# Fabstir/fabstir-vectordb

Measured on AMD Instinct MI355X. Metric: k-NN queries/sec at recall@10>=0.95, 1Mx384 f32, higher is better.
Workload: dtype f32

## Files before the change

### fabstir-vectordb_amd/csrc/fvdb_graph.cpp

```cpp
#include <algorithm>
#include <chrono>
#include <cstdio>
#include <cstdlib>
#include <cstring>
#include <map>
#include <new>
#include <string>
#include <vector>

#include "fvdb_internal.h"
#include "common.h"
#include "kernels_graph.h"
#include "kernels_graph_fast.h"
#include "kernels_graph_build.h"
#include "kernels_graph_maint.h"

using namespace fvdb;

struct fvdb_graph {
  fvdb_store* store = nullptr;
  uint32_t M = 0, M0 = 0;
  uint32_t stride0 = 0, strideU = 0;
  uint32_t n = 0, n_cap = 0;
  uint32_t u_rows = 0, u_cap = 0;
// ... 290 lines not shown
    g->tag += 1;
    hipLaunchKernelGGL(kernels.commit, dim3(1), dim3(kBuildThreads), lds, stream, v, first, n, grp.count, g->tag, 0u, nullptr, nullptr, nullptr, 1u);
    return;
  }
  for (uint32_t p = 0; p < grp.count; ++p) {
    g->tag += 1;
    hipLaunchKernelGGL(kernels.search, dim3(sched.K, kBuildLayers), dim3(kBuildThreads), lds, stream, v, first, n, sched.exact_positions,
                       g->tag, g->d_spec.as<uint32_t>(), g->d_elog.as<uint32_t>());
    hipLaunchKernelGGL(kernels.commit, dim3(1), dim3(kBuildThreads), lds, stream, v, first, n, sched.K, g->tag, sched.knobs.max_rerun,
                       g->d_spec.as<uint32_t>(), g->d_elog.as<uint32_t>(), g->d_chg.as<uint32_t>(), sched.knobs.strict);
  }
}

#ifdef FVDB_BUILD_STAMPS
void build_stamps_begin(fvdb_graph* g, BuildView* v) {
  (void)g->d_build_stamps.ensure(64 * 8);
  (void)hipMemset(g->d_build_stamps.p, 0, 64 * 8);
  v->dbg = g->d_build_stamps.as<unsigned long long>();
}
void build_stamps_print(fvdb_graph* g, const BuildState& st, uint32_t done) {
  unsigned long long h[16] = {};
  (void)hipMemcpy(h, g->d_build_stamps.p, sizeof(h), hipMemcpyDeviceToHost);
  fprintf(stderr, "[build stamps] of replay+select (us): replay %.1f  select %.1f  (table = the rest) | admissions %.1f\n", h[6] * 0.01 / std::max(1u, st.n_rerun),
          h[7] * 0.01 / std::max(1u, st.n_rerun), (double)h[8] / std::max(1u, st.n_rerun));
  const double us = 0.01, nn = std::max(1u, st.n_rerun);
  fprintf(stderr, "[build stamps] per searched insert (us): replay+select %.1f  fetch %.1f  score %.1f | greedy %.1f  all searches %.1f  links %.1f"
          " | rounds %.1f expanded %.1f scored %.0f\n", h[0] * us / nn, h[1] * us / nn, h[2] * us / nn, h[3] * us / nn, h[4] * us / nn,
          h[5] * us / std::max(1u, done), st.rounds / nn, st.consumed / nn, st.scored / nn);
}
#else
inline void build_stamps_begin(fvdb_graph*, BuildView*) {}
inline void build_stamps_print(fvdb_graph*, const BuildState&, uint32_t) {}
#endif

void report_insert(const InsertPlan& plan, const BuildState& st) {
  if (!getenv("FVDB_BUILD_DEBUG")) return;
  fprintf(stderr, "[device insert] %u linked, %u adopted, stops %u: entry %u, gave-up %u, order/strict %u, caps %u, added node nearer than a later pop %u, added node inside the final set %u, dropped node matters %u | "
          "checks %u, touched rows %u\n", st.cursor, st.n_valid, st.n_stopped, st.why[1], st.why[2], st.why[3], st.why[4], st.why[5], st.why[6],
          st.why[9], st.why[7], st.why[8]);
  fprintf(stderr, "[device insert] searches that left the register set: pops tied %u, evictions tied %u, result tied %u, heap overflow %u | speculations given up or restarted %u\n",
          st.why[11], st.why[12], st.why[13], st.why[14], st.spec_ties);
  fprintf(stderr, "[device insert] second looks: overlapping %u, nodes the popped newcomer would bring in %u, later pop is the maximum %u\n", st.why[15], st.why[16], st.why[17]);
  if (plan.repr == 2)
    fprintf(stderr, "[device insert] hashed visited set, %u slots: %u searches gave up on a full set (%u of them inserts handed to the host), "
            "entries after a search: largest %u, mean %.0f over %u searches\n", plan.slots, st.why[18], st.vis_host, st.vis_peak,
            (double)st.vis_sum / std::max(1u, st.vis_searches), st.vis_searches);
}

void fold_insert(fvdb_graph* g, const InsertPlan& plan, const BuildState& st, uint32_t launches, uint32_t* n_done,
                 fvdb_graph_insert_stats* stats) {
  if (plan.repr == 2) {
    g->ins_hashed += st.cursor;
    g->ins_vis_over += st.vis_host;
    g->ins_vis_searches += st.vis_searches;
    g->ins_vis_entries += st.vis_sum;
    g->ins_vis_peak = std::max(g->ins_vis_peak, st.vis_peak);
  }
  g->entry = st.entry;
  g->top_level = st.entry_level;
  g->has_entry = st.has_entry != 0;
  const fvdb_graph_insert_stats acc{st.cursor, st.status, st.n_valid, st.n_rerun, st.n_stopped, st.rounds, st.consumed, st.scored, st.ties, launches};
  g->last = acc;
  if (stats) *stats = acc;
  if (n_done) *n_done = st.cursor;
}

using FastKernel = decltype(&hnsw_search_fast_kernel<3, 16, true>);
template <int NB, int R>
FastKernel fast_kernel_of(bool bytemap) {
  return bytemap ? hnsw_search_fast_kernel<NB, R, true> : hnsw_search_fast_kernel<NB, R, false>;
}
FastKernel fast_kernel(uint32_t nb128, int R, bool bytemap) {
  switch (nb128) {
    case 1: return fast_kernel_of<1, 16>(bytemap);
    case 2: return fast_kernel_of<2, 16>(bytemap);
    case 3: return R == 8 ? fast_kernel_of<3, 8>(bytemap) : R == 12 ? fast_kernel_of<3, 12>(bytemap) : fast_kernel_of<3, 16>(bytemap);
    case 4: return fast_kernel_of<4, 12>(bytemap);
    case 5:
    case 6: return fast_kernel_of<6, 8>(bytemap);
    default: return fast_kernel_of<8, 6>(bytemap);
  }
}

struct SearchPlan {
  bool bytemap;
  uint32_t words, vstride, tcap, spill_cap, cand_cap;
  size_t lds;
  uint32_t wave_lds;
  FastKernel fast;
  decltype(&hnsw_search_kernel<true>) exact;
  bool rh;
};

int search_scratch(fvdb_graph* g, fvdb_ctx* ctx, uint32_t slot, uint32_t B, uint32_t ef, SearchPlan* sp) {
  sp->words = (g->n + 31) / 32;
  sp->tcap = getenv("FVDB_GRAPH_TCAP") ? std::max(1, atoi(getenv("FVDB_GRAPH_TCAP"))) : 8192;
  static const bool no_bytes = getenv("FVDB_GRAPH_BITMAP") != nullptr;
  const uint32_t vbytes = ((g->n + 63) / 64) * 64;
  sp->bytemap = !no_bytes && (uint64_t)vbytes * std::max<uint32_t>(B, 1024) <= (1ull << 30);
  sp->vstride = sp->bytemap ? vbytes : sp->words * 4;
  if (sp->words != g->vis_words || sp->tcap != g->vis_tcap || sp->vstride != g->vis_stride) {
    for (auto& v : g->vis_B) v = 0;
    g->vis_words = sp->words;
    g->vis_tcap = sp->tcap;
    g->vis_stride = sp->vstride;
  }
  if (B > g->vis_B[slot]) {
    HIPCHK(ctx, g->s_visited[slot].ensure((size_t)B * sp->vstride));
    HIPCHK(ctx, hipMemsetAsync(g->s_visited[slot].p, 0, g->s_visited[slot].cap, ctx->stream));
    HIPCHK(ctx, g->s_touched[slot].ensure((size_t)B * sp->tcap * 4));
    g->vis_B[slot] = B;
  }
  sp->spill_cap = std::min<uint32_t>(((g->n + 63) / 64) * 64, 8192);
  HIPCHK(ctx, g->s_spill[slot].ensure((size_t)B * sp->spill_cap * 8));
  const int cand_env = getenv("FVDB_GRAPH_CAND_CAP") ? atoi(getenv("FVDB_GRAPH_CAND_CAP")) : 0;
  sp->cand_cap = cand_env > 0 ? (uint32_t)cand_env : std::max<uint32_t>(1024, 8 * ef);
  sp->lds = graph_lds_bytes(g->store->dpad, ef, sp->cand_cap);
  if (sp->lds > 160 * 1024) FAIL(ctx, FVDB_E_UNSUPPORTED, "dimension / ef too large for the on-chip traversal state");
  return FVDB_OK;
}

int search_kernel(fvdb_graph* g, fvdb_ctx* ctx, uint32_t ef, SearchPlan* sp) {
  static const bool lds_heaps = getenv("FVDB_GRAPH_LDS_HEAPS") != nullptr;
  sp->rh = ef <= 63 && !lds_heaps;
  static const bool no_fast = getenv("FVDB_GRAPH_NO_FAST") != nullptr;
  static const int fast_r = getenv("FVDB_GRAPH_FAST_R") ? atoi(getenv("FVDB_GRAPH_FAST_R")) : 0;
  const uint32_t nb128 = (g->store->dpad + 127) / 128;
  if (no_fast || !sp->rh || nb128 > 8 || g->n >= 0x80000000u) {
    sp->exact = sp->rh ? hnsw_search_kernel<true> : hnsw_search_kernel<false>;
    return FVDB_OK;
  }
  int R = nb128 <= 3 ? 16 : (nb128 == 4 ? 12 : (nb128 <= 6 ? 8 : 6));
  if (nb128 == 3 && (fast_r == 8 || fast_r == 12)) R = fast_r;
  sp->wave_lds = (uint32_t)((std::max(graph_fast_lds_bytes((uint32_t)R), sp->lds) + 15) & ~(size_t)15);
  sp->lds = 4 * (size_t)sp->wave_lds;
  if (sp->lds > 160 * 1024) FAIL(ctx, FVDB_E_UNSUPPORTED, "dimension / ef too large for the on-chip traversal state");
  sp->fast = fast_kernel(nb128, R, sp->bytemap);
  return FVDB_OK;
}

#ifdef FVDB_GRAPH_STAMPS
unsigned long long* graph_stamps_report(fvdb_graph* g) {
  constexpr size_t kStampWords = 8 + 3 * 16384 + 4;
  if (!g->d_stamps.p) {
    (void)g->d_stamps.ensure(kStampWords * 8);
    (void)hipMemset(g->d_stamps.p, 0, kStampWords * 8);
  }
  unsigned long long* d_stamps = g->d_stamps.as<unsigned long long>();
  (void)hipDeviceSynchronize();
  std::vector<unsigned long long> h(kStampWords);
  (void)hipMemcpy(h.data(), d_stamps, kStampWords * 8, hipMemcpyDeviceToHost);
  fprintf(stderr, "[graph stamps, cumulative] s0 %llu s1 %llu s2 %llu s3 %llu | rows %llu rounds %llu hops %llu total %llu | score: issue %llu "
          "first-block wait+products %llu other-block products %llu adds %llu\n",
          h[0], h[1], h[2], h[3], h[4], h[5], h[6], h[7], h[8 + 3 * 16384], h[8 + 3 * 16384 + 1], h[8 + 3 * 16384 + 2], h[8 + 3 * 16384 + 3]);
  std::vector<unsigned long long> cyc, hp, rt;
  {
    std::map<unsigned, unsigned> per_cu, per_simd;
    unsigned late = 0;
    unsigned long long first = ~0ull;
    for (uint32_t q = 0; q < 16384; ++q)
      if (h[8 + 3 * q]) first = std::min(first, h[8 + 3 * q + 1]);
    for (uint32_t q = 0; q < 16384; ++q)
      if (h[8 + 3 * q]) {
        const unsigned hw = (unsigned)((h[8 + 3 * q] >> 32) & 0x0FFFFFFFu), xcc = (unsigned)(h[8 + 3 * q] >> 60);
        const unsigned cu = (xcc << 16) | (hw & 0xFF00u);
        per_cu[cu]++;
        per_simd[(cu << 2) | ((hw >> 4) & 3)]++;
        if (h[8 + 3 * q + 1] - first > 10000) late++;
        h[8 + 3 * q] &= 0xFFFFFFFFull;
      }
    unsigned mx_cu = 0, mx_simd = 0;
    for (auto& kv : per_cu) mx_cu = std::max(mx_cu, kv.second);
    for (auto& kv : per_simd) mx_simd = std::max(mx_simd, kv.second);
    fprintf(stderr, "[graph stamps, placement] CUs used %zu (max waves on one CU %u), SIMDs used %zu (max on one %u), waves starting > 100 us late: %u\n",
            per_cu.size(), mx_cu, per_simd.size(), mx_simd, late);
  }
  for (uint32_t q = 0; q < 16384; ++q)
    if (h[8 + 3 * q]) {
      cyc.push_back(h[8 + 3 * q]);
      hp.push_back(h[8 + 3 * q + 1]);
      rt.push_back(h[8 + 3 * q + 2]);
    }
  if (!cyc.empty()) {
    double csum = 0, rsum = 0;
    for (size_t i = 0; i < cyc.size(); ++i) {
      csum += (double)cyc[i];
      rsum += (double)rt[i];
    }
    unsigned long long t0 = ~0ull, t1 = 0;
    for (size_t i = 0; i < cyc.size(); ++i) {
      t0 = std::min(t0, hp[i]);
      t1 = std::max(t1, hp[i] + rt[i]);
    }
    std::vector<unsigned long long> st;
    for (size_t i = 0; i < cyc.size(); ++i) st.push_back(hp[i] - t0);
    std::sort(cyc.begin(), cyc.end());
    std::sort(st.begin(), st.end());
    std::sort(rt.begin(), rt.end());
    const size_t n = cyc.size();
    fprintf(stderr, "[graph stamps, last launch] queries %zu  cycles p50 %llu max %llu | wave lifetime us p50 %.1f p99 %.1f max %.1f | clock %.2f GHz | "
            "first start .. last end %.1f us; starts us: p25 %.1f p50 %.1f p75 %.1f p90 %.1f max %.1f\n", n, cyc[n / 2], cyc[n - 1],
            rt[n / 2] / 100.0, rt[n * 99 / 100] / 100.0, rt[n - 1] / 100.0, csum / rsum / 10.0, (t1 - t0) / 100.0, st[n / 4] / 100.0,
            st[n / 2] / 100.0, st[n * 3 / 4] / 100.0, st[n * 9 / 10] / 100.0, st[n - 1] / 100.0);
  }
  (void)hipMemset(d_stamps, 0, kStampWords * 8);
  return d_stamps;
}
#else
inline unsigned long long* graph_stamps_report(fvdb_graph*) { return nullptr; }
#endif

}
// ... 748 lines not shown
```

### fabstir-vectordb_amd/csrc/kernels_graph.h

```cpp
#pragma once
#include "common.h"
#include "wave_ops.h"

#pragma clang fp contract(off)

namespace fvdb {

struct GraphView {
  const float* rows;
  const uint32_t* level;
  const uint32_t* deleted;
  const uint32_t* adj0;
  const uint32_t* ubase;
  const uint32_t* adjU;
  uint32_t stride0, strideU;
  uint32_t n, dpad, entry, top_level;
  uint32_t any_deleted;
  unsigned long long* counters;
  unsigned long long* stamps;
};

#ifdef FVDB_GRAPH_STAMPS
#define STAMP(var) const unsigned long long var = __builtin_amdgcn_s_memtime()
#define STAMP_ADD(slot, a, b) t_acc[slot] += (b) - (a)
#else
#define STAMP(var)
#define STAMP_ADD(slot, a, b)
#endif

struct HItem {
  uint32_t node;
  float d;
};

__device__ __forceinline__ bool h_le(const HItem a, const HItem b) { return a.d >= b.d; }

__device__ __forceinline__ void h_sift_up(HItem* h, uint32_t start, uint32_t pos) {
  const HItem elt = h[pos];
  while (pos > start) {
    const uint32_t parent = (pos - 1) >> 1;
    if (h_le(elt, h[parent])) break;
    h[pos] = h[parent];
    pos = parent;
  }
  h[pos] = elt;
}
__device__ __forceinline__ void h_push(HItem* h, uint32_t& n, const HItem c) {
  h[n] = c;
  h_sift_up(h, 0, n);
  n += 1;
}
__device__ __forceinline__ HItem h_pop(HItem* h, uint32_t& n) {
  n -= 1;
  HItem item = h[n];
  if (n > 0) {
    const HItem root = h[0];
    h[0] = item;
    item = root;
    const uint32_t end = n;
    uint32_t pos = 0;
    const HItem elt = h[0];
    uint32_t child = 1;
    const uint32_t lim = end >= 2 ? end - 2 : 0;
    while (child <= lim) {
      if (h_le(h[child], h[child + 1])) child += 1;
      h[pos] = h[child];
      pos = child;
      child = 2 * pos + 1;
    }
    if (child == end - 1) {
      h[pos] = h[child];
      pos = child;
    }
    h[pos] = elt;
    h_sift_up(h, 0, pos);
  }
  return item;
}

__device__ __forceinline__ void rh_sift_up(uint32_t& hn, float& hd, uint32_t pos, uint32_t en, float ed, int lane) {
  const uint32_t x = pos + 1, y = (uint32_t)lane + 1;
  const int bx = 31 - __builtin_clz(x), by = 31 - __builtin_clz(y);
  const bool onpath = by <= bx && (x >> (bx - by)) == y;
  const bool self = (uint32_t)lane == pos;
// ... 127 lines not shown
__device__ __forceinline__ void lds_push_parallel(HItem* h, uint32_t& n, const HItem c, int lane) {
  heap_push_parallel(HeapRef{h, nullptr, 0xFFFFFFFFu}, n, c, lane);
}
__device__ __forceinline__ HItem lds_pop_parallel(HItem* h, uint32_t& n, int lane) {
  return heap_pop_parallel(HeapRef{h, nullptr, 0xFFFFFFFFu}, n, lane);
}

__device__ __forceinline__ void score_pending(const GraphView& g, const float* q_lds, float* pf_scratch,
                                              const uint32_t* pending, float* pdist, uint32_t np, int lane) {
  const uint32_t dpad = g.dpad;
  const uint32_t lpr = (dpad + 31) >> 5, nlines = np * lpr;
  for (uint32_t l = lane; l < nlines; l += 64) {
    const uint32_t r = l / lpr, ln = l - r * lpr;
    const float* src = g.rows + (size_t)pending[r] * dpad + ln * 32;
    __builtin_amdgcn_global_load_lds((const __attribute__((address_space(1))) void*)src,
                                     (__attribute__((address_space(3))) void*)pf_scratch, 4, 0, 0);
  }
  if ((uint32_t)lane < np) {
    const float* row = g.rows + (size_t)pending[lane] * dpad;
    const float4* xp = (const float4*)row;
    const float4* qp = (const float4*)q_lds;
    const uint32_t nb = dpad >> 5;
    float acc = 0.0f;
    auto issue = [&](uint32_t bi, float4 (&dst)[8]) {
      const uint32_t bb = bi < nb ? bi : nb - 1;
#pragma unroll
      for (int i = 0; i < 8; ++i) dst[i] = xp[bb * 8 + i];
    };
    auto issue_q = [&](uint32_t bi, float4 (&dst)[8]) {
      const uint32_t bb = bi < nb ? bi : nb - 1;
#pragma unroll
      for (int i = 0; i < 8; ++i) dst[i] = qp[bb * 8 + i];
    };
    auto fold = [&](const float4 (&src)[8], const float4 (&qv)[8]) {
#pragma unroll
      for (int i = 0; i < 8; ++i) {
        float t;
        t = qv[i].x - src[i].x; acc = acc + t * t;
        t = qv[i].y - src[i].y; acc = acc + t * t;
        t = qv[i].z - src[i].z; acc = acc + t * t;
        t = qv[i].w - src[i].w; acc = acc + t * t;
      }
    };
    uint32_t done = 0;
    if (nb >= 2) {
      float4 r0[8], r1[8], qa[8];
      const uint32_t nb2 = nb - nb % 2;
      issue(0, r0);
      for (uint32_t bi = 0; bi < nb2; bi += 2) {
        issue(bi + 1, r1);
        issue_q(bi, qa);
        __builtin_amdgcn_sched_barrier(0);
        fold(r0, qa);
        __builtin_amdgcn_sched_barrier(0);
        issue(bi + 2, r0);
        issue_q(bi + 1, qa);
        __builtin_amdgcn_sched_barrier(0);
        fold(r1, qa);
        __builtin_amdgcn_sched_barrier(0);
      }
      done = nb2;
    }
    for (uint32_t bi = done; bi < nb; ++bi) {
      float4 t8[8], q8[8];
      issue(bi, t8);
      issue_q(bi, q8);
      fold(t8, q8);
    }
    for (uint32_t j = nb << 5; j < dpad; j += 4) {
      const float4 xv = *(const float4*)(row + j);
      const float4 qv = *(const float4*)(q_lds + j);
      float t;
      t = qv.x - xv.x; acc = acc + t * t;
      t = qv.y - xv.y; acc = acc + t * t;
      t = qv.z - xv.z; acc = acc + t * t;
      t = qv.w - xv.w; acc = acc + t * t;
    }
    pdist[lane] = sqrtf(acc);
  }
  __builtin_amdgcn_s_waitcnt(0);
  __builtin_amdgcn_wave_barrier();
}

__host__ __device__ inline size_t graph_lds_bytes(uint32_t dpad, uint32_t ef, uint32_t cand_cap) {
  size_t b = (size_t)dpad * 4 + 64 * 4 + 64 * 4 + 64 * 4 + 16 * 4;
  b = (b + 7) & ~(size_t)7;
  b += (size_t)(ef + 2) * 8 + (size_t)(ef + 1) * 8 + (size_t)cand_cap * 8;
  return (b + 15) & ~(size_t)15;
}

template <bool RH>
__device__ __forceinline__ void hnsw_search_exact_body(const GraphView& g, const float* __restrict__ queries, uint32_t b, uint32_t k,
                                                       uint32_t ef_final, uint32_t cand_cap, uint32_t* __restrict__ vis ,
                                                       uint32_t words, uint32_t* __restrict__ tch , uint32_t tcap,
                                                       uint32_t* __restrict__ out_nodes, float* __restrict__ out_dist,
                                                       uint32_t* __restrict__ out_counts, uint32_t* __restrict__ out_status,
                                                       unsigned char* lds, int lane, HItem* __restrict__ spill = nullptr ,
                                                       uint32_t spill_cap = 0) {
  const uint32_t dpad = g.dpad;
  float* q_lds = (float*)lds;
  float* pf_scratch = q_lds + dpad;
  uint32_t* pending = (uint32_t*)(pf_scratch + 64);
  float* pdist = (float*)(pending + 64);
  uint32_t* sc = (uint32_t*)(pdist + 64);
  size_t off = ((size_t)((unsigned char*)(sc + 16) - lds) + 7) & ~(size_t)7;
  HItem* near = (HItem*)(lds + off);
  HItem* res = near + (ef_final + 2);
  HItem* cand = res + (ef_final + 1);

  for (uint32_t j = lane; j < dpad; j += 64) q_lds[j] = queries[(size_t)b * dpad + j];
  if (lane == 0) sc[2] = 0;
  __builtin_amdgcn_s_waitcnt(0);
  __builtin_amdgcn_wave_barrier();

  if (lane == 0) pending[0] = g.entry;
  __builtin_amdgcn_s_waitcnt(0);
  __builtin_amdgcn_wave_barrier();
  score_pending(g, q_lds, pf_scratch, pending, pdist, 1, lane);
  uint32_t n_res = 1;
  if (lane == 0) res[0] = HItem{g.entry, pdist[0]};
  __builtin_amdgcn_s_waitcnt(0);
  __builtin_amdgcn_wave_barrier();

#ifdef FVDB_GRAPH_STAMPS
  unsigned long long t_acc[8] = {0, 0, 0, 0, 0, 0, 0, 0};
  const unsigned long long t_begin = __builtin_amdgcn_s_memtime();
  const unsigned long long r_begin = __builtin_amdgcn_s_memrealtime();
#endif
  uint32_t rows_scored = 1, hops_done = 0;
  for (uint32_t layer = g.top_level + 1; layer-- > 0;) {
    const uint32_t ef = layer == 0 ? ef_final : 1;
    uint32_t nC = 0, nN = 0, nT = 0;
    uint32_t nr_node = 0;
    float nr_d = 0.0f;
    bool overflow = false;
    const HItem ep = res[0];
    if (RH) {
      heap_push_parallel(HeapRef{cand, spill, cand_cap}, nC, ep, lane);
      rh_push(nr_node, nr_d, nN, ep.node, -ep.d, lane);
      if (lane == 0) {
        atomicOr(&vis[ep.node >> 5], 1u << (ep.node & 31));
        tch[0] = ep.node;
      }
    } else if (lane == 0) {
      h_push(cand, nC, ep);
      h_push(near, nN, HItem{ep.node, -ep.d});
      atomicOr(&vis[ep.node >> 5], 1u << (ep.node & 31));
      tch[0] = ep.node;
    }
    nT = 1;
    for (;;) {
      STAMP(t0s);
      if (RH) {
        uint32_t stop_r = 1, node_r = 0;
        if (nC > 0) {
          const HItem cur = heap_pop_parallel(HeapRef{cand, spill, cand_cap}, nC, lane);
          stop_r = cur.d > -rlane_f(nr_d, 0) ? 1u : 0u;
          node_r = cur.node;
        }
        if (lane == 0) {
          sc[0] = stop_r;
          sc[1] = node_r;
        }
      } else if (lane == 0) {
        uint32_t stop = 0, node = 0;
        if (nC == 0) {
          stop = 1;
        } else {
          const HItem cur = h_pop(cand, nC);
          if (cur.d > -near[0].d) stop = 1;
          node = cur.node;
        }
        sc[0] = stop;
        sc[1] = node;
      }
      __builtin_amdgcn_s_waitcnt(0);
      __builtin_amdgcn_wave_barrier();
      const uint32_t stop = sc[0], node = sc[1];
      if (stop) break;
      STAMP(t1s);
      STAMP_ADD(0, t0s, t1s);
      uint32_t np = 0;
      if (layer == 0 || g.level[node] >= layer) {
        uint32_t cnt, nb = 0;
        if (layer == 0) {
          const uint32_t* row = g.adj0 + (size_t)node * g.stride0;
          const uint32_t w = row[0];
          nb = (uint32_t)lane + 1 < g.stride0 ? row[lane + 1] : 0u;
          cnt = __builtin_amdgcn_readfirstlane(w);
        } else {
          const uint32_t* row = g.adjU + (size_t)(g.ubase[node] + layer - 1) * g.strideU;
          cnt = __builtin_amdgcn_readfirstlane(row[0]);
          if ((uint32_t)lane < cnt) nb = row[lane + 1];
        }
        bool fresh = false, keep = false;
        if ((uint32_t)lane < cnt) {
          const uint32_t bit = 1u << (nb & 31);
          fresh = (atomicOr(&vis[nb >> 5], bit) & bit) == 0;
          keep = fresh && (g.any_deleted == 0 || g.deleted[nb] == 0);
        }
        const uint64_t fm = __ballot(fresh), km = __ballot(keep);
        const uint64_t lt = (1ull << lane) - 1;
        const uint32_t nf = __popcll(fm);
        if (fresh && nT + nf <= tcap) tch[nT + __popcll(fm & lt)] = nb;
        nT += nf;
        np = __popcll(km);
        if (keep) pending[__popcll(km & lt)] = nb;
      }
      if (overflow) break;
      __builtin_amdgcn_s_waitcnt(0);
      __builtin_amdgcn_wave_barrier();
      STAMP(t2s);
      STAMP_ADD(1, t1s, t2s);
      hops_done += 1;
      rows_scored += np;
      if (np) {
        score_pending(g, q_lds, pf_scratch, pending, pdist, np, lane);
        STAMP(t3s);
        STAMP_ADD(2, t2s, t3s);
#ifdef FVDB_GRAPH_STAMPS
        t_acc[4] += np;
        t_acc[5] += 1;
#endif
        if (RH) {
          const float pd = (uint32_t)lane < np ? pdist[lane] : 0.0f;
          const uint32_t pn = (uint32_t)lane < np ? pending[lane] : 0u;
          float worst = -rlane_f(nr_d, 0);
          uint64_t todo = __ballot((uint32_t)lane < np && (nN < ef || pd < worst));
          while (todo) {
            const uint32_t i = (uint32_t)__builtin_ctzll(todo);
            todo &= todo - 1;
            const float d = rlane_f(pd, i);
            if (d < worst || nN < ef) {
              if (nC >= cand_cap + spill_cap) {
                overflow = true;
                break;
              }
              const uint32_t node_i = __builtin_amdgcn_readlane(pn, i);
              heap_push_parallel(HeapRef{cand, spill, cand_cap}, nC, HItem{node_i, d}, lane);
              rh_push(nr_node, nr_d, nN, node_i, -d, lane);
              if (nN > ef) rh_pop(nr_node, nr_d, nN, lane);
              worst = -rlane_f(nr_d, 0);
            }
          }
          if (overflow && lane == 0) sc[2] = 1;
        } else {
          const uint32_t nN0 = __builtin_amdgcn_readfirstlane(nN);
          const float worst0 = -near[0].d;
          const bool maybe = (uint32_t)lane < np && (nN0 < ef || pdist[lane] < worst0);
          uint64_t todo = __ballot(maybe);
          if (lane == 0) {
            float worst = worst0;
            while (todo) {
              const uint32_t i = (uint32_t)__builtin_ctzll(todo);
              todo &= todo - 1;
              const float d = pdist[i];
              if (d < worst || nN < ef) {
                if (nC >= cand_cap) {
                  sc[2] = 1;
                  break;
                }
                h_push(cand, nC, HItem{pending[i], d});
                h_push(near, nN, HItem{pending[i], -d});
                if (nN > ef) (void)h_pop(near, nN);
                worst = -near[0].d;
              }
            }
          }
        }
        __builtin_amdgcn_s_waitcnt(0);
        __builtin_amdgcn_wave_barrier();
        STAMP(t4s);
        STAMP_ADD(3, t3s, t4s);
        if (sc[2]) {
          overflow = true;
          break;
        }
      }
#ifdef FVDB_GRAPH_STAMPS
      t_acc[6] += 1;
#endif
    }
    if (RH) {
      if ((uint32_t)lane < nN) near[lane] = HItem{nr_node, nr_d};
      if (lane == 0) sc[3] = nN;
    } else if (lane == 0) {
      sc[3] = nN;
    }
    __builtin_amdgcn_s_waitcnt(0);
    __builtin_amdgcn_wave_barrier();
    const uint32_t nn = sc[3];
    if (!overflow) {
      for (uint32_t i0 = 0; i0 < nn; i0 += 64) {
        const uint32_t i = i0 + lane;
        if (i < nn) {
          const HItem me = near[i];
          const float md = -me.d;
          uint32_t rank = 0;
          for (uint32_t j = 0; j < nn; ++j) {
            const float dj = -near[j].d;
            rank += (dj < md || (dj == md && j < i)) ? 1u : 0u;
          }
          res[rank] = HItem{me.node, md};
        }
      }
      n_res = nn;
    }
    if (nT <= tcap && !overflow) {
      for (uint32_t i = lane; i < nT; i += 64) vis[tch[i] >> 5] = 0;
    } else {
      for (uint32_t w = lane; w < words; w += 64) vis[w] = 0;
    }
    __builtin_amdgcn_s_waitcnt(0);
    __builtin_amdgcn_wave_barrier();
    if (overflow) {
      if (lane == 0) {
        out_status[b] = 1;
        out_counts[b] = 0;
      }
      return;
    }
  }
#ifdef FVDB_GRAPH_STAMPS
  if (lane == 0 && g.stamps) {
    t_acc[7] = __builtin_amdgcn_s_memtime() - t_begin;
    for (int i = 0; i < 8; ++i) atomicAdd(g.stamps + i, t_acc[i]);
    if (b < 16384) {
      const unsigned long long hw = (unsigned)__builtin_amdgcn_s_getreg((31 << 11) | 4), xcc = (unsigned)__builtin_amdgcn_s_getreg((31 << 11) | 20) & 15u;
      g.stamps[8 + 3 * b] = (t_acc[7] & 0xFFFFFFFFull) | (hw << 32) | (xcc << 60);
      g.stamps[8 + 3 * b + 1] = r_begin;
      g.stamps[8 + 3 * b + 2] = __builtin_amdgcn_s_memrealtime() - r_begin;
    }
  }
#endif
  if (lane == 0 && g.counters) {
    atomicAdd(g.counters + 0, (unsigned long long)rows_scored);
    atomicAdd(g.counters + 1, (unsigned long long)hops_done);
  }
  if (lane == 0) {
    uint32_t w = 0;
    for (uint32_t i = 0; i < n_res && w < k; ++i) {
      const HItem c = res[i];
      if (g.deleted[c.node]) continue;
      out_nodes[(size_t)b * k + w] = c.node;
      out_dist[(size_t)b * k + w] = c.d;
      ++w;
    }
    out_counts[b] = w;
    out_status[b] = 0;
    for (uint32_t i = w; i < k; ++i) {
      out_nodes[(size_t)b * k + i] = 0xFFFFFFFFu;
      out_dist[(size_t)b * k + i] = __uint_as_float(0x7F800000u);
    }
  }
}

template <bool RH>
__global__ __launch_bounds__(64) __attribute__((amdgpu_waves_per_eu(1, 3))) void hnsw_search_kernel(const GraphView g, const float* __restrict__ queries,
                                                         uint32_t B, uint32_t k, uint32_t ef_final, uint32_t cand_cap,
                                                         uint32_t* __restrict__ visited ,
                                                         uint32_t words, uint32_t* __restrict__ touched ,
                                                         uint32_t tcap, uint32_t* __restrict__ out_nodes,
                                                         float* __restrict__ out_dist, uint32_t* __restrict__ out_counts,
                                                         uint32_t* __restrict__ out_status, HItem* __restrict__ spill ,
                                                         uint32_t spill_cap) {
  extern __shared__ __attribute__((aligned(16))) unsigned char lds[];
  const uint32_t b = blockIdx.x;
  if (b >= B) return;
  hnsw_search_exact_body<RH>(g, queries, b, k, ef_final, cand_cap, visited + (size_t)b * words, words, touched + (size_t)b * tcap, tcap, out_nodes, out_dist, out_counts,
                             out_status, lds, (int)threadIdx.x, spill ? spill + (size_t)b * spill_cap : nullptr, spill ? spill_cap : 0u);
}

}
```

### fabstir-vectordb_amd/csrc/kernels_graph_fast.h

```cpp
#pragma once
#include "kernels_graph.h"
#include "score_rows.h"
#include "wave_ops.h"

#pragma clang fp contract(off)

namespace fvdb {

#ifndef FVDB_FAST_WAVES16
#define FVDB_FAST_WAVES16 3
#endif

#ifndef FVDB_FAST_TILES
#define FVDB_FAST_TILES 2
#endif
__host__ __device__ inline size_t graph_fast_lds_bytes(uint32_t R) {
  return (64 + 16) * 4 + FVDB_FAST_TILES * (size_t)R * kScoreStride * 4;
}

template <int NB, int R>
__device__ __forceinline__ float score_round(const GraphView& g, const float2 (&q2)[NB], uint32_t pn, uint32_t cnt,
                                             float* stage, int lane
#ifdef FVDB_GRAPH_STAMPS
                                             , unsigned long long* t_acc
#define FVDB_TACC , t_acc
#else
#define FVDB_TACC
#endif
) {
  const uint32_t dpad = g.dpad, tile = (uint32_t)R * kScoreStride;
  if (dpad == (uint32_t)NB * 128u) {
    if (R > 8 && cnt > 8) return score_fixed<NB, R, true, FVDB_FAST_TILES>(g.rows, dpad, q2, pn, cnt, stage, tile, lane FVDB_TACC);
    if (R > 4 && cnt > 4) return score_fixed<NB, (R < 8 ? R : 8), true, FVDB_FAST_TILES>(g.rows, dpad, q2, pn, cnt, stage, tile, lane FVDB_TACC);
    return score_fixed<NB, (R < 4 ? R : 4), true, FVDB_FAST_TILES>(g.rows, dpad, q2, pn, cnt, stage, tile, lane FVDB_TACC);
  }
  if (R > 8 && cnt > 8) return score_fixed<NB, R, false, FVDB_FAST_TILES>(g.rows, dpad, q2, pn, cnt, stage, tile, lane FVDB_TACC);
  return score_fixed<NB, (R < 8 ? R : 8), false, FVDB_FAST_TILES>(g.rows, dpad, q2, pn, cnt, stage, tile, lane FVDB_TACC);
}
#undef FVDB_TACC

template <int NB, int R, bool BYTES>
__global__ __launch_bounds__(256, (R <= 8 ? 4 : (R <= 12 ? 3 : FVDB_FAST_WAVES16))) void hnsw_search_fast_kernel(const GraphView g, const float* __restrict__ queries, uint32_t B,
                                                              uint32_t k, uint32_t ef_final, uint32_t cand_cap, uint32_t wave_lds,
                                                              uint8_t* __restrict__ visited ,
                                                              uint32_t vstride,
                                                              uint32_t words, uint32_t* __restrict__ touched ,
                                                              uint32_t tcap, uint32_t* __restrict__ out_nodes,
                                                              float* __restrict__ out_dist, uint32_t* __restrict__ out_counts,
                                                              uint32_t* __restrict__ out_status, HItem* __restrict__ spill ,
                                                              uint32_t spill_cap) {
  extern __shared__ __attribute__((aligned(16))) unsigned char lds_f_all[];
  const int lane = threadIdx.x & 63;
  const uint32_t b = blockIdx.x * 4 + (threadIdx.x >> 6);
  if (b >= B) return;
  unsigned char* lds_f = lds_f_all + (threadIdx.x >> 6) * wave_lds;
  uint32_t* pending = (uint32_t*)lds_f;
  float* stage = (float*)(pending + 64 + 16);
  uint8_t* visb = visited + (size_t)b * vstride;
  uint32_t* vis = (uint32_t*)visb;
  uint32_t* tch = touched + (size_t)b * tcap;
  const uint32_t dpad = g.dpad;
  const uint64_t lt = (1ull << lane) - 1;

  float2 q2[NB];
#pragma unroll
  for (int c = 0; c < NB; ++c) {
    const uint32_t j = (uint32_t)c * 128u + 2u * (uint32_t)lane;
    q2[c] = j < dpad ? *(const float2*)(queries + (size_t)b * dpad + j) : make_float2(0.0f, 0.0f);
  }

#ifdef FVDB_GRAPH_STAMPS
  unsigned long long t_acc[12] = {0, 0, 0, 0, 0, 0, 0, 0, 0, 0, 0, 0};
#endif
  const float d_entry = __uint_as_float(__builtin_amdgcn_readfirstlane(__float_as_uint(score_round<NB, R>(g, q2, g.entry, 1, stage, lane
#ifdef FVDB_GRAPH_STAMPS
                                                                                                            , t_acc
#endif
                                                                                                            ))));
  uint32_t ep_node = g.entry;
  float ep_d = d_entry;

#ifdef FVDB_GRAPH_STAMPS
  const unsigned long long t_begin = __builtin_amdgcn_s_memtime();
  const unsigned long long r_begin = __builtin_amdgcn_s_memrealtime();
#endif
  uint32_t rows_scored = 1, hops_done = 0;
  uint32_t hn = 0;
  float hd = 0.0f;
  uint32_t nN = 0;
  uint32_t status = 0;
  float amb = __uint_as_float(0x7FC00000u), twin_d = 0.0f;
  uint32_t twin_left = 0;
  for (uint32_t layer = g.top_level + 1; layer-- > 0 && status == 0;) {
    const uint32_t ef = layer == 0 ? ef_final : 1;
    uint32_t nT = 1;
    nN = 1;
    hn = ep_node;
    hd = ep_d;
    amb = __uint_as_float(0x7FC00000u);
    twin_left = 0;
    if (lane == 0) {
      if (BYTES) visb[ep_node] = 1;
      else atomicOr(&vis[ep_node >> 5], 1u << (ep_node & 31));
      tch[0] = ep_node;
    }
    uint32_t pf_node = 0xFFFFFFFFu, pf_w = 0, pf_nb = 0;
    for (;;) {
      STAMP(t0s);
      const uint64_t open = __ballot((uint32_t)lane < nN && (hn >> 31) == 0);
      if (open == 0) break;
      const uint32_t cl = (uint32_t)__builtin_ctzll(open);
      const uint32_t node = __builtin_amdgcn_readlane(hn, cl);
      {
        const float dc = rlane_f(hd, cl);
        const uint32_t holders = (uint32_t)__popcll(open & __ballot((uint32_t)lane < nN && hd == dc));
        if (holders > 2 || dc == amb || (twin_left != 0 && (dc != twin_d || holders != twin_left))) {
          status = 2;
          break;
        }
        if (holders == 2 && twin_left == 0) {
          twin_d = dc;
          twin_left = 2;
        }
      }
      if ((uint32_t)lane == cl) hn |= 0x80000000u;
      uint32_t np = 0;
      if (layer == 0 || g.level[node] >= layer) {
        uint32_t cnt, nb = 0;
        if (layer == 0) {
          uint32_t w;
          if (pf_node == node) {
            w = pf_w;
            nb = pf_nb;
          } else {
            const uint32_t* row = g.adj0 + (size_t)node * g.stride0;
            w = row[0];
            nb = (uint32_t)lane + 1 < g.stride0 ? row[lane + 1] : 0u;
          }
          cnt = __builtin_amdgcn_readfirstlane(w);
          const uint64_t rest = open & (open - 1);
          if (rest) {
            pf_node = __builtin_amdgcn_readlane(hn, (uint32_t)__builtin_ctzll(rest));
            const uint32_t* prow = g.adj0 + (size_t)pf_node * g.stride0;
            pf_w = prow[0];
            pf_nb = (uint32_t)lane + 1 < g.stride0 ? prow[lane + 1] : 0u;
          } else {
            pf_node = 0xFFFFFFFFu;
          }
        } else {
          const uint32_t* row = g.adjU + (size_t)(g.ubase[node] + layer - 1) * g.strideU;
          cnt = __builtin_amdgcn_readfirstlane(row[0]);
          if ((uint32_t)lane < cnt) nb = row[lane + 1];
        }
        bool fresh = false, keep = false;
        if ((uint32_t)lane < cnt) {
          if (BYTES) {
            fresh = visb[nb] == 0;
            if (fresh) visb[nb] = 1;
          } else {
            const uint32_t bit = 1u << (nb & 31);
            fresh = (atomicOr(&vis[nb >> 5], bit) & bit) == 0;
          }
          keep = fresh && (g.any_deleted == 0 || g.deleted[nb] == 0);
        }
        const uint64_t fm = __ballot(fresh), km = __ballot(keep);
        const uint32_t nf = __popcll(fm);
        if (fresh && nT + nf <= tcap) tch[nT + __popcll(fm & lt)] = nb;
        nT += nf;
        np = __popcll(km);
        if (keep) pending[__popcll(km & lt)] = nb;
      }
      if (status) break;
      hops_done += 1;
      rows_scored += np;
      __builtin_amdgcn_s_waitcnt(0xC07F);
      __builtin_amdgcn_wave_barrier();
      STAMP(t1s);
      STAMP_ADD(0, t0s, t1s);
// ... 12 lines not shown
        t_acc[4] += cnt;
        t_acc[5] += 1;
#endif
        float worst = nN ? rlane_f(hd, nN - 1) : 0.0f;
        uint64_t todo = __ballot((uint32_t)lane < cnt && (nN < ef || pd < worst));
        while (todo) {
          const uint32_t i = (uint32_t)__builtin_ctzll(todo);
          todo &= todo - 1;
          const float d = rlane_f(pd, i);
          if (nN < ef || d < worst) {
            const uint32_t nd = __builtin_amdgcn_readlane(pn, i);
            const bool mine = (uint32_t)lane < nN;
#ifdef FVDB_FAST_STRICT_TIES
            if (__ballot(mine && hd == d)) {
              status = 2;
              break;
            }
#endif
            if (twin_left != 0 && d < twin_d) {
              status = 2;
              break;
            }
            if (nN == ef) {
              const uint64_t grp = __ballot(mine && hd == worst);
              if (__popcll(grp) > 1) {
                amb = worst;
                const uint64_t ex = __ballot(mine && hd == worst && (hn >> 31) != 0);
                const uint32_t last = nN - 1;
                if (ex && ((ex >> last) & 1ull) == 0) {
                  const uint32_t l = (uint32_t)__builtin_ctzll(ex);
                  const uint32_t a = __builtin_amdgcn_readlane(hn, l), z = __builtin_amdgcn_readlane(hn, last);
                  if ((uint32_t)lane == l) hn = z;
                  if ((uint32_t)lane == last) hn = a;
                }
              }
            }
            const uint32_t pos = __popcll(__ballot(mine && hd < d));
            const uint32_t up_n = dpp_wave_shr1(hn);
            const float up_d = __uint_as_float(dpp_wave_shr1(__float_as_uint(hd)));
            if ((uint32_t)lane > pos) {
              hn = up_n;
              hd = up_d;
            } else if ((uint32_t)lane == pos) {
              hn = nd;
              hd = d;
            }
            if (nN < ef) nN += 1;
            worst = rlane_f(hd, nN - 1);
          }
        }
        STAMP(t4s);
        STAMP_ADD(2, t3s, t4s);
      }
#ifdef FVDB_GRAPH_STAMPS
      t_acc[6] += 1;
#endif
      if (status) break;
      if (twin_left != 0) twin_left -= 1;
    }
    if (status == 0) {
      const uint32_t read = layer != 0 ? 1u : (g.any_deleted ? nN : min(nN, k + 1));
      const bool in = (uint32_t)lane < read;
      const float nxt = __uint_as_float(dpp_wave_shr1(__float_as_uint(hd)));
      if (__ballot(in && lane > 0 && nxt == hd) || __ballot(in && hd == amb)) status = 2;
    }
    if (nT <= tcap && status != 1) {
      for (uint32_t i = lane; i < nT; i += 64) {
        if (BYTES) visb[tch[i]] = 0;
        else vis[tch[i] >> 5] = 0;
      }
    } else {
      for (uint32_t w = lane; w < (BYTES ? vstride / 4 : words); w += 64) vis[w] = 0;
    }
    __builtin_amdgcn_s_waitcnt(0);
    __builtin_amdgcn_wave_barrier();
    ep_node = __builtin_amdgcn_readlane(hn, 0) & 0x7FFFFFFFu;
    ep_d = rlane_f(hd, 0);
  }
  if (lane == 0 && g.counters) {
    atomicAdd(g.counters + 3, 1ull);
    if (status == 2) atomicAdd(g.counters + 2, 1ull);
  }
  if (status == 2) {
    hnsw_search_exact_body<true>(g, queries, b, k, ef_final, cand_cap, vis, words, tch, tcap, out_nodes, out_dist,
                                 out_counts, out_status, lds_f, lane, spill ? spill + (size_t)b * spill_cap : nullptr, spill ? spill_cap : 0u);
    return;
  }
  if (status) {
    if (lane == 0) {
      out_status[b] = status;
      out_counts[b] = 0;
    }
    return;
  }
#ifdef FVDB_GRAPH_STAMPS
  if (lane == 0 && g.stamps) {
    t_acc[7] = __builtin_amdgcn_s_memtime() - t_begin;
    for (int i = 0; i < 8; ++i) atomicAdd(g.stamps + i, t_acc[i]);
    for (int i = 8; i < 12; ++i) atomicAdd(g.stamps + 8 + 3 * 16384 + (i - 8), t_acc[i]);
    if (b < 16384) {
      const unsigned long long hw = (unsigned)__builtin_amdgcn_s_getreg((31 << 11) | 4), xcc = (unsigned)__builtin_amdgcn_s_getreg((31 << 11) | 20) & 15u;
      g.stamps[8 + 3 * b] = (t_acc[7] & 0xFFFFFFFFull) | (hw << 32) | (xcc << 60);
      g.stamps[8 + 3 * b + 1] = r_begin;
      g.stamps[8 + 3 * b + 2] = __builtin_amdgcn_s_memrealtime() - r_begin;
    }
  }
#endif
  if (lane == 0 && g.counters) {
    atomicAdd(g.counters + 0, (unsigned long long)rows_scored);
    atomicAdd(g.counters + 1, (unsigned long long)hops_done);
  }
  const uint32_t my = hn & 0x7FFFFFFFu;
  const bool live = (uint32_t)lane < nN && g.deleted[my] == 0;
  const uint64_t lm = __ballot(live);
  const uint32_t rank = __popcll(lm & lt), total = min(__popcll(lm), k);
  if (live && rank < k) {
    out_nodes[(size_t)b * k + rank] = my;
    out_dist[(size_t)b * k + rank] = hd;
  }
  for (uint32_t i = total + lane; i < k; i += 64) {
    out_nodes[(size_t)b * k + i] = 0xFFFFFFFFu;
    out_dist[(size_t)b * k + i] = __uint_as_float(0x7F800000u);
  }
  if (lane == 0) {
    out_counts[b] = total;
    out_status[b] = 0;
  }
}

}
```

Baseline: 1.680 million.

## Use register-resident tiled scoring in exact HNSW path and resume fallback mid-descent

The exact search body is templated on the number of 128-float blocks, so it scores pending candidates with the tiled score_fixed routine, keeping the query in registers instead of in LDS. This shrinks LDS use. When the fast kernel falls back to the exact path (status 2), it now resumes from the layer, entry node and counters it had reached instead of restarting from the top. This saves the repeated upper-layer descent and speeds up scoring in fallback cases, at the cost of more template instantiations and register pressure.

```diff
diff --git a/fabstir-vectordb_amd/csrc/fvdb_graph.cpp b/fabstir-vectordb_amd/csrc/fvdb_graph.cpp
--- a/fabstir-vectordb_amd/csrc/fvdb_graph.cpp
+++ b/fabstir-vectordb_amd/csrc/fvdb_graph.cpp
@@ -396,13 +396,32 @@
   }
 }
 
+using ExactKernel = decltype(&hnsw_search_kernel<true, 0>);
+template <int NB>
+ExactKernel exact_kernel_of(bool rh) {
+  return rh ? hnsw_search_kernel<true, NB> : hnsw_search_kernel<false, NB>;
+}
+ExactKernel exact_kernel(uint32_t nb128, bool rh) {
+  switch (nb128) {
+    case 1: return exact_kernel_of<1>(rh);
+    case 2: return exact_kernel_of<2>(rh);
+    case 3: return exact_kernel_of<3>(rh);
+    case 4: return exact_kernel_of<4>(rh);
+    case 5:
+    case 6: return exact_kernel_of<6>(rh);
+    case 7:
+    case 8: return exact_kernel_of<8>(rh);
+    default: return exact_kernel_of<0>(rh);
+  }
+}
+
 struct SearchPlan {
   bool bytemap;
   uint32_t words, vstride, tcap, spill_cap, cand_cap;
   size_t lds;
   uint32_t wave_lds;
   FastKernel fast;
-  decltype(&hnsw_search_kernel<true>) exact;
+  decltype(&hnsw_search_kernel<true, 0>) exact;
   bool rh;
 };
 
@@ -429,7 +448,7 @@
   HIPCHK(ctx, g->s_spill[slot].ensure((size_t)B * sp->spill_cap * 8));
   const int cand_env = getenv("FVDB_GRAPH_CAND_CAP") ? atoi(getenv("FVDB_GRAPH_CAND_CAP")) : 0;
   sp->cand_cap = cand_env > 0 ? (uint32_t)cand_env : std::max<uint32_t>(1024, 8 * ef);
-  sp->lds = graph_lds_bytes(g->store->dpad, ef, sp->cand_cap);
+  sp->lds = graph_lds_bytes(g->store->dpad, ef, sp->cand_cap, (g->store->dpad + 127) / 128 <= 8);
   if (sp->lds > 160 * 1024) FAIL(ctx, FVDB_E_UNSUPPORTED, "dimension / ef too large for the on-chip traversal state");
   return FVDB_OK;
 }
@@ -441,7 +460,7 @@
   static const int fast_r = getenv("FVDB_GRAPH_FAST_R") ? atoi(getenv("FVDB_GRAPH_FAST_R")) : 0;
   const uint32_t nb128 = (g->store->dpad + 127) / 128;
   if (no_fast || !sp->rh || nb128 > 8 || g->n >= 0x80000000u) {
-    sp->exact = sp->rh ? hnsw_search_kernel<true> : hnsw_search_kernel<false>;
+    sp->exact = exact_kernel(nb128, sp->rh);
     return FVDB_OK;
   }
   int R = nb128 <= 3 ? 16 : (nb128 == 4 ? 12 : (nb128 <= 6 ? 8 : 6));
diff --git a/fabstir-vectordb_amd/csrc/kernels_graph.h b/fabstir-vectordb_amd/csrc/kernels_graph.h
--- a/fabstir-vectordb_amd/csrc/kernels_graph.h
+++ b/fabstir-vectordb_amd/csrc/kernels_graph.h
@@ -1,5 +1,6 @@
 #pragma once
 #include "common.h"
+#include "score_rows.h"
 #include "wave_ops.h"
 
 #pragma clang fp contract(off)
@@ -293,15 +294,43 @@
   __builtin_amdgcn_wave_barrier();
 }
 
-__host__ __device__ inline size_t graph_lds_bytes(uint32_t dpad, uint32_t ef, uint32_t cand_cap) {
-  size_t b = (size_t)dpad * 4 + 64 * 4 + 64 * 4 + 64 * 4 + 16 * 4;
+constexpr int kExactTileRows = 8;
+template <int NB>
+constexpr int exact_round_rows() { return NB <= 4 ? kExactTileRows : 4; }
+
+template <int NB>
+__device__ __forceinline__ void score_pending_tiled(const GraphView& g, const float2 (&q2)[NB], float* tile, const uint32_t* pending,
+                                                    float* pdist, uint32_t np, int lane) {
+  constexpr int XR = exact_round_rows<NB>();
+  const uint32_t dpad = g.dpad;
+  const bool full = dpad == (uint32_t)NB * 128u;
+  for (uint32_t base = 0; base < np; base += XR) {
+    const uint32_t cnt = min((uint32_t)XR, np - base);
+    const uint32_t pn = (uint32_t)lane < cnt ? pending[base + lane] : 0u;
+    float d;
+    if (full) d = cnt > 4 ? score_fixed<NB, XR, true, 1>(g.rows, dpad, q2, pn, cnt, tile, 0, lane) : score_fixed<NB, 4, true, 1>(g.rows, dpad, q2, pn, cnt, tile, 0, lane);
+    else d = cnt > 4 ? score_fixed<NB, XR, false, 1>(g.rows, dpad, q2, pn, cnt, tile, 0, lane) : score_fixed<NB, 4, false, 1>(g.rows, dpad, q2, pn, cnt, tile, 0, lane);
+    if ((uint32_t)lane < cnt) pdist[base + lane] = d;
+  }
+  __builtin_amdgcn_s_waitcnt(0);
+  __builtin_amdgcn_wave_barrier();
+}
+
+__host__ __device__ inline size_t graph_lds_bytes(uint32_t dpad, uint32_t ef, uint32_t cand_cap, bool tiled) {
+  size_t b = (tiled ? (size_t)kExactTileRows * kScoreStride * 4 : (size_t)dpad * 4 + 64 * 4) + 64 * 4 + 64 * 4 + 16 * 4;
   b = (b + 7) & ~(size_t)7;
   b += (size_t)(ef + 2) * 8 + (size_t)(ef + 1) * 8 + (size_t)cand_cap * 8;
   return (b + 15) & ~(size_t)15;
 }
 
-template <bool RH>
-__device__ __forceinline__ void hnsw_search_exact_body(const GraphView& g, const float* __restrict__ queries, uint32_t b, uint32_t k,
+struct ExactStart {
+  uint32_t layer = 0xFFFFFFFFu, node = 0;
+  float d = 0.0f;
+  uint32_t rows = 0, hops = 0;
+};
+template <bool RH, int NB>
+__device__ __forceinline__ void hnsw_search_exact_body(const GraphView& g, const float* __restrict__ queries, const float2 (&q2)[NB ? NB : 1],
+                                                       const ExactStart start, uint32_t b, uint32_t k,
                                                        uint32_t ef_final, uint32_t cand_cap, uint32_t* __restrict__ vis ,
                                                        uint32_t words, uint32_t* __restrict__ tch , uint32_t tcap,
                                                        uint32_t* __restrict__ out_nodes, float* __restrict__ out_dist,
@@ -311,7 +340,7 @@
   const uint32_t dpad = g.dpad;
   float* q_lds = (float*)lds;
   float* pf_scratch = q_lds + dpad;
-  uint32_t* pending = (uint32_t*)(pf_scratch + 64);
+  uint32_t* pending = NB ? (uint32_t*)(q_lds + kExactTileRows * kScoreStride) : (uint32_t*)(pf_scratch + 64);
   float* pdist = (float*)(pending + 64);
   uint32_t* sc = (uint32_t*)(pdist + 64);
   size_t off = ((size_t)((unsigned char*)(sc + 16) - lds) + 7) & ~(size_t)7;
@@ -319,17 +348,27 @@
   HItem* res = near + (ef_final + 2);
   HItem* cand = res + (ef_final + 1);
 
-  for (uint32_t j = lane; j < dpad; j += 64) q_lds[j] = queries[(size_t)b * dpad + j];
+  auto score = [&](uint32_t np) {
+    if constexpr (NB != 0) score_pending_tiled<NB>(g, q2, q_lds, pending, pdist, np, lane);
+    else score_pending(g, q_lds, pf_scratch, pending, pdist, np, lane);
+  };
+  if (NB == 0)
+    for (uint32_t j = lane; j < dpad; j += 64) q_lds[j] = queries[(size_t)b * dpad + j];
   if (lane == 0) sc[2] = 0;
   __builtin_amdgcn_s_waitcnt(0);
   __builtin_amdgcn_wave_barrier();
 
-  if (lane == 0) pending[0] = g.entry;
-  __builtin_amdgcn_s_waitcnt(0);
-  __builtin_amdgcn_wave_barrier();
-  score_pending(g, q_lds, pf_scratch, pending, pdist, 1, lane);
+  const bool from_top = start.layer > g.top_level;
   uint32_t n_res = 1;
-  if (lane == 0) res[0] = HItem{g.entry, pdist[0]};
+  if (from_top) {
+    if (lane == 0) pending[0] = g.entry;
+    __builtin_amdgcn_s_waitcnt(0);
+    __builtin_amdgcn_wave_barrier();
+    score(1);
+    if (lane == 0) res[0] = HItem{g.entry, pdist[0]};
+  } else if (lane == 0) {
+    res[0] = HItem{start.node, start.d};
+  }
   __builtin_amdgcn_s_waitcnt(0);
   __builtin_amdgcn_wave_barrier();
 
@@ -338,8 +377,8 @@
   const unsigned long long t_begin = __builtin_amdgcn_s_memtime();
   const unsigned long long r_begin = __builtin_amdgcn_s_memrealtime();
 #endif
-  uint32_t rows_scored = 1, hops_done = 0;
-  for (uint32_t layer = g.top_level + 1; layer-- > 0;) {
+  uint32_t rows_scored = from_top ? 1 : start.rows, hops_done = from_top ? 0 : start.hops;
+  for (uint32_t layer = (from_top ? g.top_level : start.layer) + 1; layer-- > 0;) {
     const uint32_t ef = layer == 0 ? ef_final : 1;
     uint32_t nC = 0, nN = 0, nT = 0;
     uint32_t nr_node = 0;
@@ -426,7 +465,7 @@
       hops_done += 1;
       rows_scored += np;
       if (np) {
-        score_pending(g, q_lds, pf_scratch, pending, pdist, np, lane);
+        score(np);
         STAMP(t3s);
         STAMP_ADD(2, t2s, t3s);
 #ifdef FVDB_GRAPH_STAMPS
@@ -566,7 +605,7 @@
   }
 }
 
-template <bool RH>
+template <bool RH, int NB>
 __global__ __launch_bounds__(64) __attribute__((amdgpu_waves_per_eu(1, 3))) void hnsw_search_kernel(const GraphView g, const float* __restrict__ queries,
                                                          uint32_t B, uint32_t k, uint32_t ef_final, uint32_t cand_cap,
                                                          uint32_t* __restrict__ visited ,
@@ -578,8 +617,16 @@
   extern __shared__ __attribute__((aligned(16))) unsigned char lds[];
   const uint32_t b = blockIdx.x;
   if (b >= B) return;
-  hnsw_search_exact_body<RH>(g, queries, b, k, ef_final, cand_cap, visited + (size_t)b * words, words, touched + (size_t)b * tcap, tcap, out_nodes, out_dist, out_counts,
-                             out_status, lds, (int)threadIdx.x, spill ? spill + (size_t)b * spill_cap : nullptr, spill ? spill_cap : 0u);
-}
-
-}
+  const int lane = (int)threadIdx.x;
+  float2 q2[NB ? NB : 1];
+#pragma unroll
+  for (int c = 0; c < NB; ++c) {
+    const uint32_t j = (uint32_t)c * 128u + 2u * (uint32_t)lane;
+    q2[c] = j < g.dpad ? *(const float2*)(queries + (size_t)b * g.dpad + j) : make_float2(0.0f, 0.0f);
+  }
+  if (NB == 0) q2[0] = make_float2(0.0f, 0.0f);
+  hnsw_search_exact_body<RH, NB>(g, queries, q2, ExactStart{}, b, k, ef_final, cand_cap, visited + (size_t)b * words, words, touched + (size_t)b * tcap, tcap, out_nodes, out_dist, out_counts,
+                             out_status, lds, lane, spill ? spill + (size_t)b * spill_cap : nullptr, spill ? spill_cap : 0u);
+}
+
+}
diff --git a/fabstir-vectordb_amd/csrc/kernels_graph_fast.h b/fabstir-vectordb_amd/csrc/kernels_graph_fast.h
--- a/fabstir-vectordb_amd/csrc/kernels_graph_fast.h
+++ b/fabstir-vectordb_amd/csrc/kernels_graph_fast.h
@@ -91,9 +91,15 @@
   uint32_t status = 0;
   float amb = __uint_as_float(0x7FC00000u), twin_d = 0.0f;
   uint32_t twin_left = 0;
+  ExactStart at;
   for (uint32_t layer = g.top_level + 1; layer-- > 0 && status == 0;) {
     const uint32_t ef = layer == 0 ? ef_final : 1;
     uint32_t nT = 1;
+    at.layer = layer;
+    at.node = ep_node;
+    at.d = ep_d;
+    at.rows = rows_scored;
+    at.hops = hops_done;
     nN = 1;
     hn = ep_node;
     hd = ep_d;
@@ -272,7 +278,7 @@
     if (status == 2) atomicAdd(g.counters + 2, 1ull);
   }
   if (status == 2) {
-    hnsw_search_exact_body<true>(g, queries, b, k, ef_final, cand_cap, vis, words, tch, tcap, out_nodes, out_dist,
+    hnsw_search_exact_body<true, NB>(g, queries, q2, at, b, k, ef_final, cand_cap, vis, words, tch, tcap, out_nodes, out_dist,
                                  out_counts, out_status, lds_f, lane, spill ? spill + (size_t)b * spill_cap : nullptr, spill ? spill_cap : 0u);
     return;
   }
```

Measured after the change: 1.570 million. 0.935x the previous value.
